# qutech/filter_functions

Hardware: AMD Instinct MI355X
Metric: filter-function elements/sec (n_seg*n_omega*n_nops*d^2) at d=4 (higher is better)
Workload: dtype f64

## Files before the change

filter_functions_amd/csrc/post.hip:

```cpp
#include <algorithm>

#include <cstdlib>

#include "ffk_internal.h"

namespace ffk {
namespace {

__global__ void reduce_chunks_kernel(const cplx* __restrict__ Ypart, int chunks, size_t slab,
                                     cplx* __restrict__ Bt) {
    const size_t e = static_cast<size_t>(blockIdx.x)*blockDim.x + threadIdx.x;
    if (e >= slab) return;
    cplx acc = Ypart[e];
    for (int c = 1; c < chunks; ++c) {
        const cplx v = Ypart[static_cast<size_t>(c)*slab + e];
        acc.re += v.re;
        acc.im += v.im;
    }
    Bt[e] = acc;
}

__global__ __launch_bounds__(64) void basis_compact_kernel(const cplx* __restrict__ basis, int d,
                                                           int* __restrict__ nnz,
                                                           int* __restrict__ rows,
// ... 328 lines not shown
    const int w = blockIdx.x*blockDim.x + threadIdx.x;
    if (w >= W) return;
    for (long long ab = blockIdx.z; ab < static_cast<long long>(A)*A; ab += gridDim.z) {
        const int a = static_cast<int>(ab / A), b = static_cast<int>(ab % A);
        for (long long kl = blockIdx.y; kl < static_cast<long long>(N)*N; kl += gridDim.y) {
            const int k = static_cast<int>(kl / N), l = static_cast<int>(kl % N);
            const cplx x = R[(static_cast<size_t>(a)*N + k)*W + w];
            const cplx y = R[(static_cast<size_t>(b)*N + l)*W + w];
            const double rr = x.re*y.re;
            const double ii = x.im*y.im;
            const double ri = x.re*y.im;
            const double ir = x.im*y.re;
            cplx v;
            v.re = rr + ii;
            v.im = ri - ir;
            F[((((static_cast<size_t>(a)*A + b)*N + k)*N + l))*W + w] = v;
        }
    }
}

constexpr int kInfidSlots = 1024, kInfidThreads = 256;
constexpr int kInfidPer = kInfidSlots/kInfidThreads;

template <int J0, int JN, typename LoadF, typename LoadS>
__device__ __forceinline__ void infid_batch(int base, int W, const double* __restrict__ omega, LoadF Fat, LoadS Sat,
                                            double (&acc)[kInfidPer], double* red = nullptr) {
    const int lane = threadIdx.x & 63;
    cplx f[kInfidPer], sp[kInfidPer];
    double om[kInfidPer];
#pragma unroll
    for (int j = J0; j < J0 + JN; ++j) {
        const int w = base + static_cast<int>(threadIdx.x) + kInfidThreads*j;
        const int wc = w < W ? w : W - 1;
        f[j] = Fat(wc);
        sp[j] = Sat(wc);
        om[j] = omega[wc];
    }
#pragma unroll
    for (int j = J0; j < J0 + JN; ++j) {
        const int w = base + static_cast<int>(threadIdx.x) + kInfidThreads*j;
        const double i0 = f[j].re*sp[j].re - f[j].im*sp[j].im;
        double i1 = __shfl_down(i0, 1, 64), o1 = __shfl_down(om[j], 1, 64);
        if (lane == 63 && w + 1 < W) {
            const cplx f1 = Fat(w + 1), s1 = Sat(w + 1);
            i1 = f1.re*s1.re - f1.im*s1.im;
            o1 = omega[w + 1];
        }
        if (w < W - 1) {
            if (red != nullptr) red[threadIdx.x + kInfidThreads*j] += (i1 + i0)*(o1 - om[j]);
            else acc[j] += (i1 + i0)*(o1 - om[j]);
        }
    }
}

template <bool FROM_REGISTERS = true>
__device__ __forceinline__ void infid_finish(double* red, const double (&acc)[kInfidPer], int d, double* out) {
    static_assert(kInfidPer == 4 && kInfidThreads == 256, "the tree below is written for 4 slots per thread, 4 wavefronts");
    double sl[kInfidPer];
#pragma unroll
    for (int j = 0; j < kInfidPer; ++j) sl[j] = FROM_REGISTERS ? acc[j] : red[threadIdx.x + kInfidThreads*j];
    double x = (sl[0] + sl[2]) + (sl[1] + sl[3]);
    __syncthreads();
    red[threadIdx.x] = x;
    __syncthreads();
    if (threadIdx.x < 128) red[threadIdx.x] = x = x + red[threadIdx.x + 128];
    __syncthreads();
    if (threadIdx.x < 64) {
        x = x + red[threadIdx.x + 64];
#pragma unroll
        for (int off = 32; off > 0; off >>= 1) x = x + __shfl_down(x, off, 64);
        if (threadIdx.x == 0) *out = (x/2.0)/(2.0*3.141592653589793*d);
    }
}

template <bool SHARDED>
__device__ __forceinline__ void infid_element(const cplx* __restrict__ F, int A, int W,
                                              const cplx* __restrict__ S, int s_ndim,
                                              const double* __restrict__ omega,
                                              const int32_t* __restrict__ idx, int n_idx,
                                              int d, int shard_width,
                                              double* __restrict__ infid, const int p) {
    __shared__ double red[kInfidSlots];
    __builtin_amdgcn_s_setprio(3);
    int ia, ib;
    const cplx* Sp;
    if (s_ndim == 3) {
        ia = idx[p / n_idx];
        ib = idx[p % n_idx];
        Sp = S + static_cast<size_t>(p)*W;
    } else {
        ia = ib = idx[p];
        Sp = S + (s_ndim == 2 ? static_cast<size_t>(p)*W : 0);
    }
    const cplx* Fp = F + (static_cast<size_t>(ia)*A + ib)*(SHARDED ? shard_width : W);
    auto Fat = [&](int w) -> cplx {
        if (SHARDED) {
            const int r = w / shard_width, wl = w - r*shard_width;
            return Fp[static_cast<size_t>(r)*A*A*shard_width + wl];
        }
        return Fp[w];
    };
    auto Sat = [&](int w) -> cplx { return Sp[w]; };
    double acc[kInfidPer];
#pragma unroll
    for (int j = 0; j < kInfidPer; ++j) red[threadIdx.x + kInfidThreads*j] = 0.0;
    for (int base = 0; base < W - 1; base += kInfidSlots) {
        infid_batch<0, kInfidPer>(base, W, omega, Fat, Sat, acc, red);
        asm volatile("" ::: "memory");
    }
    infid_finish<false>(red, acc, d, infid + p);
}

template <bool SHARDED>
__global__ __launch_bounds__(kInfidThreads) void infid_kernel(const cplx* __restrict__ F, int A, int W,
                                                              const cplx* __restrict__ S, int s_ndim,
                                                              const double* __restrict__ omega,
                                                              const int32_t* __restrict__ idx, int n_idx,
                                                              int d, int shard_width,
                                                              double* __restrict__ infid) {
    infid_element<SHARDED>(F, A, W, S, s_ndim, omega, idx, n_idx, d, shard_width, infid, blockIdx.x);
}

__global__ __launch_bounds__(kInfidThreads) void infid_pulses_kernel(const cplx* __restrict__ F, int A, int W,
                                                                     const cplx* __restrict__ S, int s_ndim,
                                                                     const double* __restrict__ omega,
                                                                     const int32_t* __restrict__ idx, int n_idx,
                                                                     int d, int nout, double* __restrict__ infid) {
    const size_t q = blockIdx.y;
    infid_element<false>(F + q*A*A*W, A, W, S, s_ndim, omega, idx, n_idx, d, 0, infid + q*nout, blockIdx.x);
}
// ... 2 lines not shown
__global__ __launch_bounds__(kInfidThreads) void infid_host_spectrum_kernel(
    const cplx* __restrict__ F, int A, int W, const cplx* __restrict__ S, int s_ndim,
    const double* __restrict__ omega, const int32_t* __restrict__ idx, int n_idx, int d,
    double* __restrict__ infid) {
    __shared__ double red[kInfidSlots];
    extern __shared__ __attribute__((aligned(16))) unsigned char stage_raw[];
    cplx* sl = reinterpret_cast<cplx*>(stage_raw);
    const int p = blockIdx.x;
    int ia, ib;
    const cplx* Sp;
    if (s_ndim == 3) {
        ia = idx[p / n_idx];
        ib = idx[p % n_idx];
        Sp = S + static_cast<size_t>(p)*W;
    } else {
        ia = ib = idx[p];
        Sp = S + (s_ndim == 2 ? static_cast<size_t>(p)*W : 0);
    }
    const cplx* Fp = F + (static_cast<size_t>(ia)*A + ib)*W;
    constexpr int kLoads = kInfidStage/kInfidThreads + 1;
    double acc[kInfidPer];
#pragma unroll
    for (int j = 0; j < kInfidPer; ++j) acc[j] = 0.0;
    for (int s0 = 0; s0 < W - 1; s0 += kInfidStage) {
        const int n = min(kInfidStage + 1, W - s0);
        cplx v[kLoads];
#pragma unroll
        for (int k = 0; k < kLoads; ++k) {
            const int i = threadIdx.x + kInfidThreads*k;
            v[k] = i < n ? Sp[s0 + i] : cplx{0.0, 0.0};
        }
#pragma unroll
        for (int k = 0; k < kLoads; ++k) {
            const int i = threadIdx.x + kInfidThreads*k;
            if (i < n) sl[i] = v[k];
        }
        __syncthreads();
        auto Fat = [&](int w) -> cplx { return Fp[w]; };
        auto Sat = [&](int w) -> cplx { return sl[w - s0]; };
        const int bend = min(W - 1, s0 + kInfidStage);
        for (int base = s0; base < bend; base += kInfidSlots) infid_batch<0, kInfidPer>(base, W, omega, Fat, Sat, acc);
        __syncthreads();
    }
    infid_finish(red, acc, d, infid + p);
}

}

hipError_t launch_reduce_chunks(const cplx* Ypart, int chunks, size_t slab, cplx* Bt,
                                hipStream_t stream) {
    const int block = 256;
    hipLaunchKernelGGL(reduce_chunks_kernel, dim3(static_cast<unsigned>((slab + block - 1)/block)),
                       dim3(block), 0, stream, Ypart, chunks, slab, Bt);
    return hipGetLastError();
}

size_t expand_workspace_bytes(int N, int d) {
    const size_t dd = static_cast<size_t>(d)*d;
    return align_up(sizeof(int)*N) + align_up(sizeof(int)*N*dd) + align_up(sizeof(cplx)*N*dd);
}

namespace {
struct CompactWs {
    int* nnz;
// ... 41 lines not shown
    const cplx* b = Ypart + static_cast<size_t>(a)*dd*W + w;
    const int n = nnz[k];
    const int* rk = rows + static_cast<size_t>(k)*dd;
    const cplx* vk = vals + static_cast<size_t>(k)*dd;
    auto summed = [&](int e) {
        cplx acc = b[static_cast<size_t>(e)*W];
        for (int z = 1; z < chunks; ++z) {
            const cplx v = b[z*slab + static_cast<size_t>(e)*W];
            acc.re += v.re;
            acc.im += v.im;
        }
        return acc;
    };
    cplx acc0 = {0.0, 0.0}, acc1 = {0.0, 0.0};
    int q = 0;
    for (; q + 1 < n; q += 2) {
        cmac(acc0, vk[q], summed(rk[q]));
        cmac(acc1, vk[q + 1], summed(rk[q + 1]));
    }
    if (q < n) cmac(acc0, vk[q], summed(rk[q]));
    R[(static_cast<size_t>(a)*N + k)*W + w] = {acc0.re + acc1.re, acc0.im + acc1.im};
}

__device__ __forceinline__ void expand_ff_tile(const cplx* __restrict__ Ypart, int chunks, size_t slab,
                                               const int* __restrict__ nnz, const int* __restrict__ rows,
                                               const cplx* __restrict__ vals, int N, int dd, int W, int A,
                                               int kt, cplx* __restrict__ R, cplx* __restrict__ F) {
    extern __shared__ __attribute__((aligned(16))) unsigned char lds_raw[];
    cplx* rl = reinterpret_cast<cplx*>(lds_raw);
    __builtin_amdgcn_s_setprio(3);
    cplx* ys = rl + static_cast<size_t>(A)*N*16;
    const int wl = threadIdx.x & 15;
    const int kl = (threadIdx.x >> 4) % kt, al = (threadIdx.x >> 4) / kt;
    const int at = (blockDim.x >> 4) / kt;
    const int w = blockIdx.x*16 + wl;
    const int wc = w < W ? w : W - 1;
    for (int idx = threadIdx.x >> 4; idx < A*dd; idx += blockDim.x >> 4) {
        const cplx* b = Ypart + static_cast<size_t>(idx)*W + wc;
        cplx acc = b[0];
        for (int z = 1; z < chunks; ++z) {
            const cplx v = b[z*slab];
            acc.re += v.re;
            acc.im += v.im;
        }
        ys[static_cast<size_t>(idx)*16 + wl] = acc;
    }
    __syncthreads();
    for (int a = al; a < A; a += at) {
        const cplx* ya = ys + static_cast<size_t>(a)*dd*16 + wl;
        for (int k = kl; k < N; k += kt) {
            const int n = nnz[k];
            const int* rk = rows + static_cast<size_t>(k)*dd;
            const cplx* vk = vals + static_cast<size_t>(k)*dd;
            auto summed = [&](int e) { return ya[e*16]; };
            cplx acc0 = {0.0, 0.0}, acc1 = {0.0, 0.0};
            int q = 0;
            for (; q + 1 < n; q += 2) {
                cmac(acc0, vk[q], summed(rk[q]));
                cmac(acc1, vk[q + 1], summed(rk[q + 1]));
            }
            if (q < n) cmac(acc0, vk[q], summed(rk[q]));
            const cplx r = {acc0.re + acc1.re, acc0.im + acc1.im};
            rl[(static_cast<size_t>(a)*N + k)*16 + wl] = r;
            if (w < W) R[(static_cast<size_t>(a)*N + k)*W + w] = r;
        }
    }
    __syncthreads();
    if (w >= W) return;
    const int npairs = A*(A + 1)/2;
    const int lanes = blockDim.x >> 4;
    for (int p = threadIdx.x >> 4; p < npairs; p += lanes) {
        int a = 0, rem = p;
        while (rem >= A - a) {
            rem -= A - a;
            ++a;
        }
        const int b = a + rem;
        const cplx* ra = rl + static_cast<size_t>(a)*N*16 + wl;
        const cplx* rb = rl + static_cast<size_t>(b)*N*16 + wl;
        cplx acc = {0.0, 0.0};
        for (int k = 0; k < N; ++k) cmac_conj(acc, ra[k*16], rb[k*16]);
        if (a == b) acc.im = 0.0;
        F[(static_cast<size_t>(a)*A + b)*W + w] = acc;
        if (a != b) F[(static_cast<size_t>(b)*A + a)*W + w] = {acc.re, -acc.im};
    }
}

__global__ __launch_bounds__(256) void expand_ff_kernel(const cplx* __restrict__ Ypart, int chunks,
                                                         size_t slab, const int* __restrict__ nnz,
// ... 5 lines not shown
}

__global__ __launch_bounds__(256) void expand_ff_pulses_kernel(const cplx* __restrict__ Ypart, int chunks,
                                                                size_t slab, const int* __restrict__ nnz,
                                                                const int* __restrict__ rows,
                                                                const cplx* __restrict__ vals, int N, int dd,
                                                                int W, int A, int kt, cplx* __restrict__ R,
                                                                cplx* __restrict__ F) {
    const size_t p = blockIdx.y;
    expand_ff_tile(Ypart + p*chunks*slab, chunks, slab, nnz, rows, vals, N, dd, W, A, kt,
                   R + p*A*N*W, F + p*A*A*W);
}

bool expand_ff_supported(int A, int N) {
    return static_cast<size_t>(A)*2*N*16*sizeof(cplx) <= 128*1024;
}

hipError_t launch_expand_ff(const cplx* Ypart, int chunks, size_t slab, int A, int N, int d, int W,
                            cplx* R, cplx* F, void* ws, hipStream_t stream) {
    if (!expand_ff_supported(A, N)) return hipErrorInvalidValue;
    const CompactWs cw = slice_compact_ws(ws, N, d);
    const int kt = N >= 16 ? 16 : (N >= 8 ? 8 : 4);
    const int at = std::max(1, std::min(A, 16/kt));
    const size_t lds = static_cast<size_t>(A)*(N + d*d)*16*sizeof(cplx);
    if (lds > 160*1024) return hipErrorInvalidValue;
    if (lds > 48*1024) {
        hipError_t err = hipFuncSetAttribute(reinterpret_cast<const void*>(expand_ff_kernel),
                                             hipFuncAttributeMaxDynamicSharedMemorySize,
                                             static_cast<int>(lds));
        if (err != hipSuccess) return err;
    }
    hipLaunchKernelGGL(expand_ff_kernel, dim3((W + 15)/16), dim3(16*kt*at), lds, stream, Ypart,
                       chunks, slab, cw.nnz, cw.rows, cw.vals, N, d*d, W, A, kt, R, F);
    return hipGetLastError();
}

hipError_t launch_expand_ff_pulses(const cplx* Ypart, int chunks, size_t slab, int A, int N, int d, int W,
                                   int P, cplx* R, cplx* F, void* ws, hipStream_t stream) {
    if (!expand_ff_supported(A, N) || P < 1 || P > 65535) return hipErrorInvalidValue;
    const CompactWs cw = slice_compact_ws(ws, N, d);
    const int kt = N >= 16 ? 16 : (N >= 8 ? 8 : 4);
    const int at = std::max(1, std::min(A, 16/kt));
    const size_t lds = static_cast<size_t>(A)*(N + d*d)*16*sizeof(cplx);
    if (lds > 160*1024) return hipErrorInvalidValue;
    if (lds > 48*1024) {
        hipError_t err = hipFuncSetAttribute(reinterpret_cast<const void*>(expand_ff_pulses_kernel),
                                             hipFuncAttributeMaxDynamicSharedMemorySize,
                                             static_cast<int>(lds));
        if (err != hipSuccess) return err;
    }
    hipLaunchKernelGGL(expand_ff_pulses_kernel, dim3((W + 15)/16, P), dim3(16*kt*at), lds, stream, Ypart,
                       chunks, slab, cw.nnz, cw.rows, cw.vals, N, d*d, W, A, kt, R, F);
    return hipGetLastError();
}

__global__ __launch_bounds__(256) void expand_lds_kernel(const cplx* __restrict__ Ypart, int chunks,
                                                         size_t slab, const int* __restrict__ nnz,
                                                         const int* __restrict__ rows,
                                                         const cplx* __restrict__ vals, int N, int dd,
                                                         int W, cplx* __restrict__ R, int want_sparse) {
    extern __shared__ __attribute__((aligned(16))) unsigned char lds_raw[];
    if (want_sparse >= 0 && basis_is_sparse(nnz, N, dd) != (want_sparse != 0)) return;
    cplx* yl = reinterpret_cast<cplx*>(lds_raw);
    const int wl = threadIdx.x & 15, kl = threadIdx.x >> 4;
    const int a = blockIdx.y;
    const int w = blockIdx.x*16 + wl;
// ... 140 lines not shown
}

hipError_t launch_filter_function_weighted(const cplx* R, int A, int N, int W, const cplx* M,
                                           double scale, cplx* F, hipStream_t stream) {
    const int block = 128;
    hipLaunchKernelGGL(ff_weighted_kernel,
                       dim3((W + block - 1)/block, grid_axis(static_cast<long long>(A)*A)),
                       dim3(block), 0, stream, R, A, N, W, M, scale, F);
    return hipGetLastError();
}

size_t infidelity_workspace_bytes(int W, int n_idx, int s_ndim) {
    (void)W;
    (void)n_idx;
    (void)s_ndim;
    return 256;
}

hipError_t launch_infidelity_pulses(const cplx* F, int A, int W, int P, const cplx* S, int s_ndim,
                                    const double* omega, const int32_t* idx, int n_idx, int d, double* infid,
                                    hipStream_t stream) {
    const int nout = s_ndim == 3 ? n_idx*n_idx : n_idx;
    if (P < 1 || P > 65535) return hipErrorInvalidValue;
    hipLaunchKernelGGL(infid_pulses_kernel, dim3(nout, P), dim3(kInfidThreads), 0, stream, F, A, W, S, s_ndim,
                       omega, idx, n_idx, d, nout, infid);
    return hipGetLastError();
}

hipError_t launch_infidelity(const cplx* F, int A, int W, const cplx* S, int s_ndim,
                             const double* omega, const int32_t* idx, int n_idx, int d,
                             int shard_width, double* infid, void* ws, hipStream_t stream,
                             bool spectrum_on_host) {
    (void)ws;
    const int nout = s_ndim == 3 ? n_idx*n_idx : n_idx;
    if (spectrum_on_host && (shard_width <= 0 || shard_width >= W)) {
        const int lds = static_cast<int>(sizeof(cplx))*(kInfidStage + 1);
        hipError_t err = hipFuncSetAttribute(reinterpret_cast<const void*>(infid_host_spectrum_kernel),
                                             hipFuncAttributeMaxDynamicSharedMemorySize, lds);
        if (err != hipSuccess) return err;
        hipLaunchKernelGGL(infid_host_spectrum_kernel, dim3(nout), dim3(kInfidThreads), lds, stream, F, A, W, S,
                           s_ndim, omega, idx, n_idx, d, infid);
        return hipGetLastError();
    }
    if (shard_width > 0 && shard_width < W)
        hipLaunchKernelGGL(infid_kernel<true>, dim3(nout), dim3(kInfidThreads), 0, stream, F, A, W, S, s_ndim, omega,
                           idx, n_idx, d, shard_width, infid);
    else
        hipLaunchKernelGGL(infid_kernel<false>, dim3(nout), dim3(kInfidThreads), 0, stream, F, A, W, S, s_ndim, omega,
                           idx, n_idx, d, shard_width, infid);
    return hipGetLastError();
}

}
```

filter_functions_amd/csrc/prep.hip:

```cpp
#include "ffk_internal.h"

namespace ffk {
namespace {

template <int D>
__device__ void prologue_segment(const cplx (*V)[D], cplx (*Q)[D], cplx (*T)[D], cplx (*BV)[D],
                                 int g, int lane, const double* __restrict__ eigvals,
                                 const cplx* __restrict__ n_opers,
                                 const double* __restrict__ n_coeffs,
                                 const double* __restrict__ dt, const double* __restrict__ t, int G,
                                 int A, double* __restrict__ segtab, cplx* __restrict__ Tc,
                                 cplx* __restrict__ ops, cplx* __restrict__ n_opers_transformed,
                                 cplx* __restrict__ eigvecs_propagated, bool with_noise_ops = true,
                                 cplx* __restrict__ wfold = nullptr) {
    constexpr int S = seg_stride(D);
    double* st = segtab + static_cast<size_t>(g)*S;
    if (lane == 0) {
        st[0] = dt[g];
        st[1] = t[g];
    }
    cplx eb = {1.0, 0.0};
    for (int e = lane; e < D*D; e += 64) {
        const double dE = eigvals[static_cast<size_t>(g)*D + e / D] - eigvals[static_cast<size_t>(g)*D + e % D];
        double sb, cb;
        sincos_pi(0.5*(dE*dt[g]), &sb, &cb);
        st[seg_rec(e)] = dE;
        st[seg_rec(e) + 1] = sb;
        st[seg_rec(e) + 2] = cb;
        st[seg_rec(e) + 3] = 0.0;
        eb = {cb, sb};
    }
    if (lane < 2) st[2 + lane] = 0.0;
    for (int e = 4 + 4*D*D + lane; e < S; e += 64) st[e] = 0.0;

    for (int e = lane; e < D*D; e += 64) {
        const int m = e / D, j = e % D;
        cplx acc = {0.0, 0.0};
#pragma unroll
        for (int k = 0; k < D; ++k) cmac_conj(acc, V[k][m], Q[k][j]);
        T[m][j] = acc;
        Tc[static_cast<size_t>(g)*D*D + e] = {acc.re, -acc.im};
        ops[static_cast<size_t>(g)*(1 + A)*D*D + e] = acc;
        if (eigvecs_propagated)
            eigvecs_propagated[static_cast<size_t>(g)*D*D + j*D + m] = {acc.re, -acc.im};
    }
    __syncthreads();

    if (!with_noise_ops) return;
    const bool fold = D == 4 && wfold != nullptr;
    if (fold) {
        if (lane < D*D) Q[lane / D][lane % D] = eb;
        __syncthreads();
    }
    for (int a = 0; a < A; ++a) {
        const cplx* B = n_opers + static_cast<size_t>(a)*D*D;
        const double s = n_coeffs ? n_coeffs[static_cast<size_t>(a)*G + g] : 1.0;
        for (int e = lane; e < D*D; e += 64) {
            const int i = e / D, n = e % D;
            cplx acc = {0.0, 0.0};
#pragma unroll
            for (int k = 0; k < D; ++k) cmac(acc, B[i*D + k], V[k][n]);
            BV[i][n] = acc;
        }
        __syncthreads();
        cplx bbar = {0.0, 0.0};
        for (int e = lane; e < D*D; e += 64) {
            const int m = e / D, n = e % D;
            cplx acc = {0.0, 0.0};
#pragma unroll
            for (int k = 0; k < D; ++k) cmac_conj(acc, V[k][m], BV[k][n]);
            acc.re *= s;
            acc.im *= s;
            ops[(static_cast<size_t>(g)*(1 + A) + 1 + a)*D*D + e] = acc;
            if (n_opers_transformed)
                n_opers_transformed[(static_cast<size_t>(a)*G + g)*D*D + e] = acc;
            if (fold) bbar = acc;
        }
        __syncthreads();
        if (fold) {
            if (lane < D*D) BV[lane / D][lane % D] = bbar;
            __syncthreads();
            if constexpr (D == 4) {
                const int m = lane >> 4, n = (lane >> 2) & 3, j = lane & 3;
                const cplx et = cmul(Q[m][n], T[n][j]);
                const cplx w = cmul(BV[m][n], et);
                wfold[(static_cast<size_t>(g)*A + a)*64 + n*16 + m*4 + j] = w;
// ... 71 lines not shown
        const int i = e / D, n = e % D;
        cplx acc = {0.0, 0.0};
#pragma unroll
        for (int k = 0; k < D; ++k) cmac(acc, B[i*D + k], V[k][n]);
        BV[i][n] = acc;
    }
    __syncthreads();
    for (int e = lane; e < D*D; e += 64) {
        const int m = e / D, n = e % D;
        cplx acc = {0.0, 0.0};
#pragma unroll
        for (int k = 0; k < D; ++k) cmac_conj(acc, V[k][m], BV[k][n]);
        acc.re *= s;
        acc.im *= s;
        ops[(static_cast<size_t>(g)*(1 + A) + 1 + a)*D*D + e] = acc;
        if (n_opers_transformed)
            n_opers_transformed[(static_cast<size_t>(a)*G + g)*D*D + e] = acc;
    }
}

constexpr int kNoiseOpsKernelMinD = 12;
inline bool split_noise_ops(int d, int A) { return d >= kNoiseOpsKernelMinD && A >= 2 && A <= 65535; }

template <int D>
__device__ __forceinline__ void apply_prologue_segment(
    const cplx* __restrict__ Qloc, const cplx* __restrict__ totals, int G, int L,
    cplx* __restrict__ Qout, const double* __restrict__ eigvals, const cplx* __restrict__ eigvecs,
    const cplx* __restrict__ n_opers, const double* __restrict__ n_coeffs,
    const double* __restrict__ dt, const double* __restrict__ t, int A,
    double* __restrict__ segtab, cplx* __restrict__ Tc, cplx* __restrict__ ops,
    bool with_noise_ops, cplx* __restrict__ wfold, const int g) {
    __builtin_amdgcn_s_setprio(3);
    __shared__ cplx E[2][D][D];
    __shared__ cplx M[D][D];
    __shared__ cplx V[D][D];
    __shared__ cplx Q[D][D];
    __shared__ cplx T[D][D];
    __shared__ cplx BV[D][D];
    constexpr int kBatch = 16;
    constexpr bool kTree = D <= 8;
    extern __shared__ __attribute__((aligned(16))) unsigned char tot_raw[];
    cplx (*tot)[D][D] = reinterpret_cast<cplx (*)[D][D]>(tot_raw);
    const int lane = threadIdx.x;
    const int c = g / L;
    for (int e = lane; e < D*D; e += 64) E[0][e / D][e % D] = {(e / D == e % D) ? 1.0 : 0.0, 0.0};
    int b = 0;
    if constexpr (kTree) {
        constexpr int DD = D*D, PER = 64/DD;
        for (int e = lane; e < c*DD; e += 64) (&tot[0][0][0])[e] = totals[e];
        __syncthreads();
        int n = c;
        while (n > 1) {
            const int pairs = n >> 1;
            for (int j0 = 0; j0 < pairs; j0 += PER) {
                const int jj = j0 + lane/DD, e = lane % DD, i = e / D, k = e % D;
                const bool act = lane < PER*DD && jj < pairs;
                cplx acc = {0.0, 0.0};
                if (act) {
#pragma unroll
                    for (int x = 0; x < D; ++x) cmac(acc, tot[2*jj + 1][i][x], tot[2*jj][x][k]);
                }
                __syncthreads();
                if (act) tot[jj][i][k] = acc;
                __syncthreads();
            }
            if (n & 1) {
                const cplx* from = &tot[n - 1][0][0] + (lane < DD ? lane : 0);
                const double carry_re = from->re, carry_im = from->im;
                __syncthreads();
                if (lane < DD) (&tot[pairs][0][0])[lane] = {carry_re, carry_im};
                __syncthreads();
            }
// ... 3 lines not shown
            for (int e = lane; e < DD; e += 64) E[0][e / D][e % D] = tot[0][e / D][e % D];
            __syncthreads();
        }
    } else {
    for (int kb = 0; kb < c; kb += kBatch) {
        const int nb = min(kBatch, c - kb);
        __syncthreads();
        for (int e = lane; e < nb*D*D; e += 64)
            (&tot[0][0][0])[e] = totals[static_cast<size_t>(kb)*D*D + e];
        __syncthreads();
        for (int k = 0; k < nb; ++k) {
            for (int e = lane; e < D*D; e += 64) {
                const int i = e / D, j = e % D;
                cplx acc = {0.0, 0.0};
#pragma unroll
                for (int x = 0; x < D; ++x) cmac(acc, tot[k][i][x], E[b][x][j]);
                E[b ^ 1][i][j] = acc;
            }
            __syncthreads();
            b ^= 1;
        }
    }
    }
    for (int e = lane; e < D*D; e += 64) M[e / D][e % D] = Qloc[static_cast<size_t>(g + 1)*D*D + e];
    if (g == 0)
        for (int e = lane; e < D*D; e += 64) Qout[e] = {(e / D == e % D) ? 1.0 : 0.0, 0.0};
    __syncthreads();
    for (int e = lane; e < D*D; e += 64) {
        const int i = e / D, j = e % D;
        cplx acc = {0.0, 0.0};
#pragma unroll
        for (int x = 0; x < D; ++x) cmac(acc, M[i][x], E[b][x][j]);
        Qout[static_cast<size_t>(g + 1)*D*D + e] = acc;
    }
    if (segtab == nullptr) return;
    __syncthreads();
    if (g % L == 0) {
        for (int e = lane; e < D*D; e += 64) Q[e / D][e % D] = E[b][e / D][e % D];
    } else {
        for (int e = lane; e < D*D; e += 64) M[e / D][e % D] = Qloc[static_cast<size_t>(g)*D*D + e];
        __syncthreads();
        for (int e = lane; e < D*D; e += 64) {
            const int i = e / D, j = e % D;
            cplx acc = {0.0, 0.0};
#pragma unroll
            for (int x = 0; x < D; ++x) cmac(acc, M[i][x], E[b][x][j]);
            Q[i][j] = acc;
        }
    }
    for (int e = lane; e < D*D; e += 64) V[e / D][e % D] = eigvecs[static_cast<size_t>(g)*D*D + e];
    __syncthreads();
    prologue_segment<D>(V, Q, T, BV, g, lane, eigvals, n_opers, n_coeffs, dt, t, G, A, segtab, Tc,
                        ops, nullptr, nullptr, with_noise_ops, wfold);
}

template <int D>
__global__ __launch_bounds__(64) void apply_prologue_kernel(
    const cplx* __restrict__ Qloc, const cplx* __restrict__ totals, int G, int L,
    cplx* __restrict__ Qout, const double* __restrict__ eigvals, const cplx* __restrict__ eigvecs,
    const cplx* __restrict__ n_opers, const double* __restrict__ n_coeffs,
    const double* __restrict__ dt, const double* __restrict__ t, int A,
    double* __restrict__ segtab, cplx* __restrict__ Tc, cplx* __restrict__ ops,
    const cplx* __restrict__ basis, int* __restrict__ nnz, int* __restrict__ rows,
    cplx* __restrict__ vals, bool with_noise_ops, cplx* __restrict__ wfold) {
    if (static_cast<int>(blockIdx.x) >= G) {
        basis_compact_one(basis, D, static_cast<int>(blockIdx.x) - G, threadIdx.x, nnz, rows, vals);
        return;
    }
    apply_prologue_segment<D>(Qloc, totals, G, L, Qout, eigvals, eigvecs, n_opers, n_coeffs, dt, t, A, segtab, Tc,
                              ops, with_noise_ops, wfold, blockIdx.x);
}

template <int D>
__global__ __launch_bounds__(64) void apply_prologue_pulses_kernel(
    const cplx* __restrict__ Qloc, const cplx* __restrict__ totals, int G, int L, int nchunks,
    cplx* __restrict__ Qout, const double* __restrict__ eigvals, const cplx* __restrict__ eigvecs,
// ... 135 lines not shown
        FFK_CASE(2) FFK_CASE(3) FFK_CASE(4) FFK_CASE(5) FFK_CASE(6) FFK_CASE(7) FFK_CASE(8)
#undef FFK_CASE
        default:
            return hipErrorInvalidValue;
    }
    return hipGetLastError();
}

hipError_t launch_apply_prologue_compact(const cplx* Qloc, const cplx* totals, int G, int d, cplx* Q,
                                         const double* eigvals, const cplx* eigvecs,
                                         const cplx* n_opers, const double* n_coeffs,
                                         const double* dt, const double* t, int A, double* segtab,
                                         cplx* Tc, cplx* ops, const cplx* basis, int N, void* ews,
                                         hipStream_t stream, cplx* wfold) {
    const int L = front_chunk(d);
    int* nnz = nullptr;
    int* rows = nullptr;
    cplx* vals = nullptr;
    int extra = 0;
    if (basis) {
        expand_workspace_slices(ews, N, d, &nnz, &rows, &vals);
        extra = N;
    }
    switch (d) {
#define FFK_CASE(D)                                                                              \
    case D:                                                                                      \
        if (D > 8) {    \
            hipError_t e = hipFuncSetAttribute(reinterpret_cast<const void*>(apply_prologue_kernel<D>), \
                                               hipFuncAttributeMaxDynamicSharedMemorySize,       \
                                               static_cast<int>(sizeof(cplx)*D*D*16));           \
            if (e != hipSuccess) return e;                                                       \
        }                                                                                        \
        hipLaunchKernelGGL(apply_prologue_kernel<D>, dim3(G + extra), dim3(64),                  \
                           sizeof(cplx)*D*D*(D <= 8 ? (G + L - 1)/L : 16), stream, Qloc,         \
                           totals, G, L, Q, eigvals, eigvecs, n_opers, n_coeffs, dt, t, A,       \
                           segtab, Tc, ops, basis, nnz, rows, vals, !split_noise_ops(D, A),      \
                           D == 4 ? wfold : nullptr);                                            \
        if (split_noise_ops(D, A))                                                               \
            hipLaunchKernelGGL(noise_ops_kernel<D>, dim3(G, A), dim3(64), 0, stream, eigvecs,    \
                               n_opers, n_coeffs, G, A, ops, nullptr);                           \
        break;
        FFK_CASE(2) FFK_CASE(3) FFK_CASE(4) FFK_CASE(5) FFK_CASE(6) FFK_CASE(7) FFK_CASE(8)
        FFK_CASE(9) FFK_CASE(10) FFK_CASE(11) FFK_CASE(12) FFK_CASE(13) FFK_CASE(14)
        FFK_CASE(15) FFK_CASE(16)
#undef FFK_CASE
        default:
            return hipErrorInvalidValue;
    }
    if (d == 8 && wfold != nullptr) return launch_fold_w8(segtab, ops, G, A, wfold, stream);
    return hipGetLastError();
}

hipError_t launch_apply_prologue_compact_pulses(const cplx* Qloc, const cplx* totals, int G, int P, int d,
                                                cplx* Q, const double* eigvals, const cplx* eigvecs,
                                                const cplx* n_opers, const double* n_coeffs, const double* dt,
                                                const double* t, int A, double* segtab, cplx* Tc, cplx* ops,
                                                const cplx* basis, int N, void* ews, hipStream_t stream,
                                                cplx* wfold) {
    const int L = front_chunk(d);
    const int nchunks = (G + L - 1)/L;
    if (P < 1 || P > 65535 || !basis) return hipErrorInvalidValue;
    int* nnz = nullptr;
    int* rows = nullptr;
    cplx* vals = nullptr;
    expand_workspace_slices(ews, N, d, &nnz, &rows, &vals);
    switch (d) {
#define FFK_CASE(D)                                                                              \
    case D:                                                                                      \
        if (D > 8) {                                                                             \
            hipError_t e = hipFuncSetAttribute(reinterpret_cast<const void*>(apply_prologue_pulses_kernel<D>), \
                                               hipFuncAttributeMaxDynamicSharedMemorySize,       \
                                               static_cast<int>(sizeof(cplx)*D*D*16));           \
            if (e != hipSuccess) return e;                                                       \
        }                                                                                        \
        hipLaunchKernelGGL(apply_prologue_pulses_kernel<D>, dim3(G + N, P), dim3(64),            \
                           sizeof(cplx)*D*D*(D <= 8 ? nchunks : 16), stream, Qloc, totals, G, L, \
                           nchunks, Q, eigvals, eigvecs, n_opers, n_coeffs, dt, t, A, segtab, Tc, \
                           ops, basis, nnz, rows, vals, D == 4 ? wfold : nullptr);               \
        break;
        FFK_CASE(2) FFK_CASE(3) FFK_CASE(4) FFK_CASE(5) FFK_CASE(6) FFK_CASE(7) FFK_CASE(8)
        FFK_CASE(9) FFK_CASE(10) FFK_CASE(11) FFK_CASE(12) FFK_CASE(13) FFK_CASE(14)
        FFK_CASE(15) FFK_CASE(16)
#undef FFK_CASE
        default:
            return hipErrorInvalidValue;
    }
    if (d == 8 && wfold != nullptr) return launch_fold_w8(segtab, ops, P*G, A, wfold, stream);
    return hipGetLastError();
}

hipError_t launch_apply_prologue(const cplx* Qloc, const cplx* totals, int G, int d, cplx* Q,
                                 const double* eigvals, const cplx* eigvecs, const cplx* n_opers,
                                 const double* n_coeffs, const double* dt, const double* t, int A,
                                 double* segtab, cplx* Tc, cplx* ops, hipStream_t stream) {
    return launch_apply_prologue_compact(Qloc, totals, G, d, Q, eigvals, eigvecs, n_opers, n_coeffs,
                                         dt, t, A, segtab, Tc, ops, nullptr, 0, nullptr, stream);
}

hipError_t launch_basis_transformed(const cplx* Tc, const cplx* basis, int G, int N, int d,
// ... 31 lines not shown
```

Before: 880.1 billion.

## Batch global loads ahead and stage sparse lists and boundaries in LDS

```diff
diff --git a/filter_functions_amd/csrc/post.hip b/filter_functions_amd/csrc/post.hip
--- a/filter_functions_amd/csrc/post.hip
+++ b/filter_functions_amd/csrc/post.hip
@@ -374,33 +374,59 @@
 constexpr int kInfidSlots = 1024, kInfidThreads = 256;
 constexpr int kInfidPer = kInfidSlots/kInfidThreads;
 
-template <int J0, int JN, typename LoadF, typename LoadS>
+__device__ __forceinline__ double infid_integrand(const cplx f, const cplx s) { return f.re*s.re - f.im*s.im; }
+
+constexpr int kInfidBoundary = 2*2*17;
+
+template <typename LoadF, typename LoadS>
 __device__ __forceinline__ void infid_batch(int base, int W, const double* __restrict__ omega, LoadF Fat, LoadS Sat,
-                                            double (&acc)[kInfidPer], double* red = nullptr) {
+                                            double (&acc)[kInfidPer], double* bnd, double* red = nullptr) {
+    static_assert(kInfidPer == 4 && kInfidThreads == 256, "16 boundary points: 4 slots x 4 wavefronts");
     const int lane = threadIdx.x & 63;
+    const int wave = static_cast<int>(threadIdx.x) >> 6;
     cplx f[kInfidPer], sp[kInfidPer];
-    double om[kInfidPer];
-#pragma unroll
-    for (int j = J0; j < J0 + JN; ++j) {
+    double om[kInfidPer], i0[kInfidPer];
+#pragma unroll
+    for (int j = 0; j < kInfidPer; ++j) {
         const int w = base + static_cast<int>(threadIdx.x) + kInfidThreads*j;
         const int wc = w < W ? w : W - 1;
         f[j] = Fat(wc);
         sp[j] = Sat(wc);
         om[j] = omega[wc];
     }
-#pragma unroll
-    for (int j = J0; j < J0 + JN; ++j) {
-        const int w = base + static_cast<int>(threadIdx.x) + kInfidThreads*j;
-        const double i0 = f[j].re*sp[j].re - f[j].im*sp[j].im;
-        double i1 = __shfl_down(i0, 1, 64), o1 = __shfl_down(om[j], 1, 64);
-        if (lane == 63 && w + 1 < W) {
-            const cplx f1 = Fat(w + 1), s1 = Sat(w + 1);
-            i1 = f1.re*s1.re - f1.im*s1.im;
-            o1 = omega[w + 1];
-        }
-        if (w < W - 1) {
-            if (red != nullptr) red[threadIdx.x + kInfidThreads*j] += (i1 + i0)*(o1 - om[j]);
-            else acc[j] += (i1 + i0)*(o1 - om[j]);
+    __builtin_amdgcn_sched_barrier(0);
+    const int par = (base/kInfidSlots) & 1;
+    double* mine = bnd + par*34 + 2*wave;
+#pragma unroll
+    for (int j = 0; j < kInfidPer; ++j) {
+        i0[j] = infid_integrand(f[j], sp[j]);
+        if (lane == 0) {
+            mine[8*j] = i0[j];
+            mine[8*j + 1] = om[j];
+        }
+    }
+    __syncthreads();
+    const bool last = threadIdx.x == kInfidThreads - 1;
+    if (last && base > 0) {
+        const double* prev = mine + (par ? -34 : 34);
+        const double i1 = mine[-6], o1 = mine[-5], ic = prev[26], oc = prev[27];
+        if (red != nullptr) red[threadIdx.x + kInfidThreads*(kInfidPer - 1)] += (i1 + ic)*(o1 - oc);
+        else acc[kInfidPer - 1] += (i1 + ic)*(o1 - oc);
+    }
+    const int left = W - 1 - base - static_cast<int>(threadIdx.x);
+#pragma unroll
+    for (int j = 0; j < kInfidPer; ++j) {
+        double i1 = __shfl_down(i0[j], 1, 64), o1 = __shfl_down(om[j], 1, 64);
+        if (lane == 63) {
+            i1 = mine[8*j + 2];
+            o1 = mine[8*j + 3];
+        }
+        if (j == kInfidPer - 1 && last) {
+            mine[26] = i0[j];
+            mine[27] = om[j];
+        } else if (kInfidThreads*j < left) {
+            if (red != nullptr) red[threadIdx.x + kInfidThreads*j] += (i1 + i0[j])*(o1 - om[j]);
+            else acc[j] += (i1 + i0[j])*(o1 - om[j]);
         }
     }
 }
@@ -433,6 +459,8 @@
                                               int d, int shard_width,
                                               double* __restrict__ infid, const int p) {
     __shared__ double red[kInfidSlots];
+    extern __shared__ __attribute__((aligned(16))) unsigned char bnd_raw[];
+    double* bnd = reinterpret_cast<double*>(bnd_raw);
     __builtin_amdgcn_s_setprio(3);
     int ia, ib;
     const cplx* Sp;
@@ -456,8 +484,8 @@
     double acc[kInfidPer];
 #pragma unroll
     for (int j = 0; j < kInfidPer; ++j) red[threadIdx.x + kInfidThreads*j] = 0.0;
-    for (int base = 0; base < W - 1; base += kInfidSlots) {
-        infid_batch<0, kInfidPer>(base, W, omega, Fat, Sat, acc, red);
+    for (int base = 0; base < W; base += kInfidSlots) {
+        infid_batch(base, W, omega, Fat, Sat, acc, bnd, red);
         asm volatile("" ::: "memory");
     }
     infid_finish<false>(red, acc, d, infid + p);
@@ -506,7 +534,8 @@
     double acc[kInfidPer];
 #pragma unroll
     for (int j = 0; j < kInfidPer; ++j) acc[j] = 0.0;
-    for (int s0 = 0; s0 < W - 1; s0 += kInfidStage) {
+    double* bnd = red + kInfidThreads;
+    for (int s0 = 0; s0 < W; s0 += kInfidStage) {
         const int n = min(kInfidStage + 1, W - s0);
         cplx v[kLoads];
 #pragma unroll
@@ -522,8 +551,8 @@
         __syncthreads();
         auto Fat = [&](int w) -> cplx { return Fp[w]; };
         auto Sat = [&](int w) -> cplx { return sl[w - s0]; };
-        const int bend = min(W - 1, s0 + kInfidStage);
-        for (int base = s0; base < bend; base += kInfidSlots) infid_batch<0, kInfidPer>(base, W, omega, Fat, Sat, acc);
+        const int bend = min(W, s0 + kInfidStage);
+        for (int base = s0; base < bend; base += kInfidSlots) infid_batch(base, W, omega, Fat, Sat, acc, bnd);
         __syncthreads();
     }
     infid_finish(red, acc, d, infid + p);
@@ -611,6 +640,11 @@
     R[(static_cast<size_t>(a)*N + k)*W + w] = {acc0.re + acc1.re, acc0.im + acc1.im};
 }
 
+__host__ __device__ constexpr bool expand_ff_lists_in_lds(int N, int dd) { return N*dd <= 1024; }
+__host__ __device__ constexpr size_t expand_ff_lds_bytes(int A, int N, int dd) {
+    return static_cast<size_t>(A)*(N + dd)*16*sizeof(cplx) +
+           (expand_ff_lists_in_lds(N, dd) ? static_cast<size_t>(N)*dd*(sizeof(cplx) + sizeof(int)) + sizeof(int)*N : 0);
+}
 __device__ __forceinline__ void expand_ff_tile(const cplx* __restrict__ Ypart, int chunks, size_t slab,
                                                const int* __restrict__ nnz, const int* __restrict__ rows,
                                                const cplx* __restrict__ vals, int N, int dd, int W, int A,
@@ -624,36 +658,93 @@
     const int at = (blockDim.x >> 4) / kt;
     const int w = blockIdx.x*16 + wl;
     const int wc = w < W ? w : W - 1;
-    for (int idx = threadIdx.x >> 4; idx < A*dd; idx += blockDim.x >> 4) {
-        const cplx* b = Ypart + static_cast<size_t>(idx)*W + wc;
-        cplx acc = b[0];
-        for (int z = 1; z < chunks; ++z) {
-            const cplx v = b[z*slab];
-            acc.re += v.re;
-            acc.im += v.im;
-        }
-        ys[static_cast<size_t>(idx)*16 + wl] = acc;
+    const bool lists_staged = expand_ff_lists_in_lds(N, dd);
+    const int nl = N*dd;
+    cplx* vals_l = ys + static_cast<size_t>(A)*dd*16;
+    int* rows_l = reinterpret_cast<int*>(vals_l + nl);
+    int* nnz_l = rows_l + nl;
+    const int tid = threadIdx.x, nthreads = blockDim.x;
+    int row0 = 0, nnz0 = 0;
+    double val0_re = 0.0, val0_im = 0.0;
+    if (lists_staged) {
+        const int e = tid < nl ? tid : nl - 1;
+        row0 = rows[e];
+        val0_re = vals[e].re;
+        val0_im = vals[e].im;
+        nnz0 = nnz[tid < N ? tid : N - 1];
+    }
+    {
+        constexpr int kFly = 8;
+        const int groups = nthreads >> 4, g0 = tid >> 4, entries = A*dd;
+        const int ne = (entries + groups - 1)/groups;
+        const int total = ne*chunks;
+        int li = 0, lz = 0;
+        int si = 0, sz = 0;
+        double acc_re = 0.0, acc_im = 0.0;
+        for (int q0 = 0; q0 < total; q0 += kFly) {
+            cplx v[kFly];
+#pragma unroll
+            for (int u = 0; u < kFly; ++u) {
+                const int idx = min(g0 + li*groups, entries - 1);
+                v[u] = Ypart[lz*slab + static_cast<size_t>(idx)*W + wc];
+                if (q0 + u + 1 < total) {
+                    if (++lz == chunks) {
+                        lz = 0;
+                        ++li;
+                    }
+                }
+            }
+#pragma unroll
+            for (int u = 0; u < kFly; ++u) {
+                if (q0 + u < total) {
+                    acc_re = sz == 0 ? v[u].re : acc_re + v[u].re;
+                    acc_im = sz == 0 ? v[u].im : acc_im + v[u].im;
+                    if (++sz == chunks) {
+                        const int idx = g0 + si*groups;
+                        if (idx < entries) ys[static_cast<size_t>(idx)*16 + wl] = {acc_re, acc_im};
+                        sz = 0;
+                        ++si;
+                    }
+                }
+            }
+        }
+    }
+    if (lists_staged) {
+        if (tid < nl) {
+            rows_l[tid] = row0;
+            vals_l[tid] = {val0_re, val0_im};
+        }
+        if (tid < N) nnz_l[tid] = nnz0;
+        for (int e = tid + nthreads; e < nl; e += nthreads) {
+            rows_l[e] = rows[e];
+            vals_l[e] = vals[e];
+        }
+        for (int e = tid + nthreads; e < N; e += nthreads) nnz_l[e] = nnz[e];
     }
     __syncthreads();
-    for (int a = al; a < A; a += at) {
-        const cplx* ya = ys + static_cast<size_t>(a)*dd*16 + wl;
-        for (int k = kl; k < N; k += kt) {
-            const int n = nnz[k];
-            const int* rk = rows + static_cast<size_t>(k)*dd;
-            const cplx* vk = vals + static_cast<size_t>(k)*dd;
-            auto summed = [&](int e) { return ya[e*16]; };
-            cplx acc0 = {0.0, 0.0}, acc1 = {0.0, 0.0};
-            int q = 0;
-            for (; q + 1 < n; q += 2) {
-                cmac(acc0, vk[q], summed(rk[q]));
-                cmac(acc1, vk[q + 1], summed(rk[q + 1]));
+    auto expand = [&](const int* __restrict__ nz, const int* __restrict__ rw, const cplx* __restrict__ vl) {
+        for (int a = al; a < A; a += at) {
+            const cplx* ya = ys + static_cast<size_t>(a)*dd*16 + wl;
+            for (int k = kl; k < N; k += kt) {
+                const int n = nz[k];
+                const int* rk = rw + static_cast<size_t>(k)*dd;
+                const cplx* vk = vl + static_cast<size_t>(k)*dd;
+                auto summed = [&](int e) { return ya[e*16]; };
+                cplx acc0 = {0.0, 0.0}, acc1 = {0.0, 0.0};
+                int q = 0;
+                for (; q + 1 < n; q += 2) {
+                    cmac(acc0, vk[q], summed(rk[q]));
+                    cmac(acc1, vk[q + 1], summed(rk[q + 1]));
+                }
+                if (q < n) cmac(acc0, vk[q], summed(rk[q]));
+                const cplx r = {acc0.re + acc1.re, acc0.im + acc1.im};
+                rl[(static_cast<size_t>(a)*N + k)*16 + wl] = r;
+                if (w < W) R[(static_cast<size_t>(a)*N + k)*W + w] = r;
             }
-            if (q < n) cmac(acc0, vk[q], summed(rk[q]));
-            const cplx r = {acc0.re + acc1.re, acc0.im + acc1.im};
-            rl[(static_cast<size_t>(a)*N + k)*16 + wl] = r;
-            if (w < W) R[(static_cast<size_t>(a)*N + k)*W + w] = r;
-        }
-    }
+        }
+    };
+    if (lists_staged) expand(nnz_l, rows_l, vals_l);
+    else expand(nnz, rows, vals);
     __syncthreads();
     if (w >= W) return;
     const int npairs = A*(A + 1)/2;
@@ -705,7 +796,7 @@
     const CompactWs cw = slice_compact_ws(ws, N, d);
     const int kt = N >= 16 ? 16 : (N >= 8 ? 8 : 4);
     const int at = std::max(1, std::min(A, 16/kt));
-    const size_t lds = static_cast<size_t>(A)*(N + d*d)*16*sizeof(cplx);
+    const size_t lds = expand_ff_lds_bytes(A, N, d*d);
     if (lds > 160*1024) return hipErrorInvalidValue;
     if (lds > 48*1024) {
         hipError_t err = hipFuncSetAttribute(reinterpret_cast<const void*>(expand_ff_kernel),
@@ -724,7 +815,7 @@
     const CompactWs cw = slice_compact_ws(ws, N, d);
     const int kt = N >= 16 ? 16 : (N >= 8 ? 8 : 4);
     const int at = std::max(1, std::min(A, 16/kt));
-    const size_t lds = static_cast<size_t>(A)*(N + d*d)*16*sizeof(cplx);
+    const size_t lds = expand_ff_lds_bytes(A, N, d*d);
     if (lds > 160*1024) return hipErrorInvalidValue;
     if (lds > 48*1024) {
         hipError_t err = hipFuncSetAttribute(reinterpret_cast<const void*>(expand_ff_pulses_kernel),
@@ -911,8 +1002,8 @@
                                     hipStream_t stream) {
     const int nout = s_ndim == 3 ? n_idx*n_idx : n_idx;
     if (P < 1 || P > 65535) return hipErrorInvalidValue;
-    hipLaunchKernelGGL(infid_pulses_kernel, dim3(nout, P), dim3(kInfidThreads), 0, stream, F, A, W, S, s_ndim,
-                       omega, idx, n_idx, d, nout, infid);
+    hipLaunchKernelGGL(infid_pulses_kernel, dim3(nout, P), dim3(kInfidThreads), kInfidBoundary*sizeof(double), stream,
+                       F, A, W, S, s_ndim, omega, idx, n_idx, d, nout, infid);
     return hipGetLastError();
 }
 
@@ -932,12 +1023,12 @@
         return hipGetLastError();
     }
     if (shard_width > 0 && shard_width < W)
-        hipLaunchKernelGGL(infid_kernel<true>, dim3(nout), dim3(kInfidThreads), 0, stream, F, A, W, S, s_ndim, omega,
-                           idx, n_idx, d, shard_width, infid);
+        hipLaunchKernelGGL(infid_kernel<true>, dim3(nout), dim3(kInfidThreads), kInfidBoundary*sizeof(double), stream,
+                           F, A, W, S, s_ndim, omega, idx, n_idx, d, shard_width, infid);
     else
-        hipLaunchKernelGGL(infid_kernel<false>, dim3(nout), dim3(kInfidThreads), 0, stream, F, A, W, S, s_ndim, omega,
-                           idx, n_idx, d, shard_width, infid);
-    return hipGetLastError();
-}
-
-}
+        hipLaunchKernelGGL(infid_kernel<false>, dim3(nout), dim3(kInfidThreads), kInfidBoundary*sizeof(double), stream,
+                           F, A, W, S, s_ndim, omega, idx, n_idx, d, shard_width, infid);
+    return hipGetLastError();
+}
+
+}
diff --git a/filter_functions_amd/csrc/prep.hip b/filter_functions_amd/csrc/prep.hip
--- a/filter_functions_amd/csrc/prep.hip
+++ b/filter_functions_amd/csrc/prep.hip
@@ -4,7 +4,7 @@
 namespace {
 
 template <int D>
-__device__ void prologue_segment(const cplx (*V)[D], cplx (*Q)[D], cplx (*T)[D], cplx (*BV)[D],
+__device__ __forceinline__ void prologue_segment(const cplx (*V)[D], cplx (*Q)[D], cplx (*T)[D], cplx (*BV)[D],
                                  int g, int lane, const double* __restrict__ eigvals,
                                  const cplx* __restrict__ n_opers,
                                  const double* __restrict__ n_coeffs,
@@ -12,18 +12,25 @@
                                  int A, double* __restrict__ segtab, cplx* __restrict__ Tc,
                                  cplx* __restrict__ ops, cplx* __restrict__ n_opers_transformed,
                                  cplx* __restrict__ eigvecs_propagated, bool with_noise_ops = true,
-                                 cplx* __restrict__ wfold = nullptr) {
+                                 cplx* __restrict__ wfold = nullptr, const bool ahead = false,
+                                 const double ev_m = 0.0, const double ev_n = 0.0, const double dt_g = 0.0,
+                                 const double t_g = 0.0, const unsigned ops_off = 0) {
+    extern __shared__ __attribute__((aligned(16))) unsigned char ahead_raw[];
+    const cplx* ops_l = reinterpret_cast<const cplx*>(ahead_raw + ops_off);
+    const double* coeffs_l = reinterpret_cast<const double*>(ops_l + static_cast<size_t>(A)*D*D);
     constexpr int S = seg_stride(D);
     double* st = segtab + static_cast<size_t>(g)*S;
+    const double dtg = ahead ? dt_g : dt[g];
     if (lane == 0) {
-        st[0] = dt[g];
-        st[1] = t[g];
+        st[0] = dtg;
+        st[1] = ahead ? t_g : t[g];
     }
     cplx eb = {1.0, 0.0};
     for (int e = lane; e < D*D; e += 64) {
-        const double dE = eigvals[static_cast<size_t>(g)*D + e / D] - eigvals[static_cast<size_t>(g)*D + e % D];
+        const double dE = ahead ? ev_m - ev_n
+                                : eigvals[static_cast<size_t>(g)*D + e / D] - eigvals[static_cast<size_t>(g)*D + e % D];
         double sb, cb;
-        sincos_pi(0.5*(dE*dt[g]), &sb, &cb);
+        sincos_pi(0.5*(dE*dtg), &sb, &cb);
         st[seg_rec(e)] = dE;
         st[seg_rec(e) + 1] = sb;
         st[seg_rec(e) + 2] = cb;
@@ -53,15 +60,19 @@
         __syncthreads();
     }
     for (int a = 0; a < A; ++a) {
-        const cplx* B = n_opers + static_cast<size_t>(a)*D*D;
-        const double s = n_coeffs ? n_coeffs[static_cast<size_t>(a)*G + g] : 1.0;
-        for (int e = lane; e < D*D; e += 64) {
-            const int i = e / D, n = e % D;
-            cplx acc = {0.0, 0.0};
-#pragma unroll
-            for (int k = 0; k < D; ++k) cmac(acc, B[i*D + k], V[k][n]);
-            BV[i][n] = acc;
-        }
+        const double s = ahead ? coeffs_l[a]
+                               : (n_coeffs ? n_coeffs[static_cast<size_t>(a)*G + g] : 1.0);
+        auto times_v = [&](const cplx* __restrict__ B) {
+            for (int e = lane; e < D*D; e += 64) {
+                const int i = e / D, n = e % D;
+                cplx acc = {0.0, 0.0};
+#pragma unroll
+                for (int k = 0; k < D; ++k) cmac(acc, B[i*D + k], V[k][n]);
+                BV[i][n] = acc;
+            }
+        };
+        if (ahead) times_v(ops_l + static_cast<size_t>(a)*D*D);
+        else times_v(n_opers + static_cast<size_t>(a)*D*D);
         __syncthreads();
         cplx bbar = {0.0, 0.0};
         for (int e = lane; e < D*D; e += 64) {
@@ -179,6 +190,13 @@
 constexpr int kNoiseOpsKernelMinD = 12;
 inline bool split_noise_ops(int d, int A) { return d >= kNoiseOpsKernelMinD && A >= 2 && A <= 65535; }
 
+__host__ __device__ constexpr bool prologue_noise_ops_in_lds(int d, int A) { return d <= 8 && A >= 1 && A*d*d <= 1024; }
+inline size_t apply_prologue_lds_bytes(int d, int nchunks, int A, bool with_noise_ops) {
+    const size_t dd = static_cast<size_t>(d)*d;
+    return sizeof(cplx)*dd*(d <= 8 ? nchunks : 16) +
+           (with_noise_ops && prologue_noise_ops_in_lds(d, A) ? sizeof(cplx)*dd*A + sizeof(double)*A : 0);
+}
+
 template <int D>
 __device__ __forceinline__ void apply_prologue_segment(
     const cplx* __restrict__ Qloc, const cplx* __restrict__ totals, int G, int L,
@@ -196,15 +214,70 @@
     __shared__ cplx BV[D][D];
     constexpr int kBatch = 16;
     constexpr bool kTree = D <= 8;
+    constexpr int kDD = D*D;
+    constexpr int kTotAhead = 4;
     extern __shared__ __attribute__((aligned(16))) unsigned char tot_raw[];
     cplx (*tot)[D][D] = reinterpret_cast<cplx (*)[D][D]>(tot_raw);
     const int lane = threadIdx.x;
     const int c = g / L;
+    const bool ahead_ops = kTree && segtab != nullptr && with_noise_ops && prologue_noise_ops_in_lds(D, A);
+    double ev_m = 0.0, ev_n = 0.0, dt_g = 0.0, t_g = 0.0;
+    if constexpr (kTree) {
+        const int e = lane < kDD ? lane : kDD - 1;
+        const int ntot = c*kDD;
+        double q0_re = 0.0, q0_im = 0.0, vv_re = 0.0, vv_im = 0.0;
+        double op0_re = 0.0, op0_im = 0.0, co0 = 1.0;
+        double tot_re[kTotAhead], tot_im[kTotAhead];
+#pragma unroll
+        for (int k = 0; k < kTotAhead; ++k) {
+            const int x = lane + 64*k;
+            const cplx* src = totals + (x < ntot ? x : (ntot > 0 ? ntot - 1 : 0));
+            tot_re[k] = src->re;
+            tot_im[k] = src->im;
+        }
+        const double q1_re = Qloc[static_cast<size_t>(g + 1)*kDD + e].re;
+        const double q1_im = Qloc[static_cast<size_t>(g + 1)*kDD + e].im;
+        cplx* ops_l = reinterpret_cast<cplx*>(tot_raw) + static_cast<size_t>((G + L - 1)/L)*kDD;
+        double* co_l = reinterpret_cast<double*>(ops_l + static_cast<size_t>(A)*kDD);
+        if (segtab != nullptr) {
+            q0_re = Qloc[static_cast<size_t>(g)*kDD + e].re;
+            q0_im = Qloc[static_cast<size_t>(g)*kDD + e].im;
+            vv_re = eigvecs[static_cast<size_t>(g)*kDD + e].re;
+            vv_im = eigvecs[static_cast<size_t>(g)*kDD + e].im;
+            ev_m = eigvals[static_cast<size_t>(g)*D + e / D];
+            ev_n = eigvals[static_cast<size_t>(g)*D + e % D];
+            dt_g = dt[g];
+            t_g = t[g];
+            if (ahead_ops) {
+                op0_re = n_opers[lane < A*kDD ? lane : A*kDD - 1].re;
+                op0_im = n_opers[lane < A*kDD ? lane : A*kDD - 1].im;
+                if (n_coeffs) co0 = n_coeffs[static_cast<size_t>(lane < A ? lane : A - 1)*G + g];
+            }
+        }
+        asm volatile("" :: "v"(tot_re[0]), "v"(tot_im[0]), "v"(tot_re[1]), "v"(tot_im[1]), "v"(tot_re[2]),
+                     "v"(tot_im[2]), "v"(tot_re[3]), "v"(tot_im[3]), "v"(q1_re), "v"(q1_im), "v"(q0_re), "v"(q0_im),
+                     "v"(vv_re), "v"(vv_im), "v"(op0_re), "v"(op0_im), "v"(co0), "v"(ev_m), "v"(ev_n), "s"(dt_g),
+                     "s"(t_g));
+#pragma unroll
+        for (int k = 0; k < kTotAhead; ++k)
+            if (lane + 64*k < ntot) (&tot[0][0][0])[lane + 64*k] = {tot_re[k], tot_im[k]};
+        if (lane < kDD) {
+            M[lane / D][lane % D] = {q1_re, q1_im};
+            T[lane / D][lane % D] = {q0_re, q0_im};
+            V[lane / D][lane % D] = {vv_re, vv_im};
+        }
+        if (ahead_ops) {
+            if (lane < A*kDD) ops_l[lane] = {op0_re, op0_im};
+            if (lane < A) co_l[lane] = co0;
+            for (int x = lane + 64; x < A*kDD; x += 64) ops_l[x] = n_opers[x];
+            for (int x = lane + 64; x < A; x += 64) co_l[x] = n_coeffs ? n_coeffs[static_cast<size_t>(x)*G + g] : 1.0;
+        }
+    }
     for (int e = lane; e < D*D; e += 64) E[0][e / D][e % D] = {(e / D == e % D) ? 1.0 : 0.0, 0.0};
     int b = 0;
     if constexpr (kTree) {
         constexpr int DD = D*D, PER = 64/DD;
-        for (int e = lane; e < c*DD; e += 64) (&tot[0][0][0])[e] = totals[e];
+        for (int e = lane + 64*kTotAhead; e < c*DD; e += 64) (&tot[0][0][0])[e] = totals[e];
         __syncthreads();
         int n = c;
         while (n > 1) {
@@ -254,7 +327,8 @@
         }
     }
     }
-    for (int e = lane; e < D*D; e += 64) M[e / D][e % D] = Qloc[static_cast<size_t>(g + 1)*D*D + e];
+    if constexpr (!kTree)
+        for (int e = lane; e < D*D; e += 64) M[e / D][e % D] = Qloc[static_cast<size_t>(g + 1)*D*D + e];
     if (g == 0)
         for (int e = lane; e < D*D; e += 64) Qout[e] = {(e / D == e % D) ? 1.0 : 0.0, 0.0};
     __syncthreads();
@@ -270,7 +344,8 @@
     if (g % L == 0) {
         for (int e = lane; e < D*D; e += 64) Q[e / D][e % D] = E[b][e / D][e % D];
     } else {
-        for (int e = lane; e < D*D; e += 64) M[e / D][e % D] = Qloc[static_cast<size_t>(g)*D*D + e];
+        for (int e = lane; e < D*D; e += 64)
+            M[e / D][e % D] = kTree ? T[e / D][e % D] : Qloc[static_cast<size_t>(g)*D*D + e];
         __syncthreads();
         for (int e = lane; e < D*D; e += 64) {
             const int i = e / D, j = e % D;
@@ -280,10 +355,17 @@
             Q[i][j] = acc;
         }
     }
-    for (int e = lane; e < D*D; e += 64) V[e / D][e % D] = eigvecs[static_cast<size_t>(g)*D*D + e];
-    __syncthreads();
-    prologue_segment<D>(V, Q, T, BV, g, lane, eigvals, n_opers, n_coeffs, dt, t, G, A, segtab, Tc,
-                        ops, nullptr, nullptr, with_noise_ops, wfold);
+    if constexpr (!kTree)
+        for (int e = lane; e < D*D; e += 64) V[e / D][e % D] = eigvecs[static_cast<size_t>(g)*D*D + e];
+    __syncthreads();
+    if constexpr (kTree) {
+        prologue_segment<D>(V, Q, T, BV, g, lane, eigvals, n_opers, n_coeffs, dt, t, G, A, segtab, Tc,
+                            ops, nullptr, nullptr, with_noise_ops, wfold, ahead_ops, ev_m, ev_n, dt_g, t_g,
+                            static_cast<unsigned>(sizeof(cplx)*((G + L - 1)/L)*kDD));
+    } else {
+        prologue_segment<D>(V, Q, T, BV, g, lane, eigvals, n_opers, n_coeffs, dt, t, G, A, segtab, Tc,
+                            ops, nullptr, nullptr, with_noise_ops, wfold);
+    }
 }
 
 template <int D>
@@ -465,17 +547,18 @@
         expand_workspace_slices(ews, N, d, &nnz, &rows, &vals);
         extra = N;
     }
+    const size_t lds_bytes = apply_prologue_lds_bytes(d, (G + L - 1)/L, A, !split_noise_ops(d, A));
     switch (d) {
 #define FFK_CASE(D)                                                                              \
     case D:                                                                                      \
-        if (D > 8) {    \
+         \
+        if (D > 8 || lds_bytes > 48*1024) {                                                      \
             hipError_t e = hipFuncSetAttribute(reinterpret_cast<const void*>(apply_prologue_kernel<D>), \
                                                hipFuncAttributeMaxDynamicSharedMemorySize,       \
-                                               static_cast<int>(sizeof(cplx)*D*D*16));           \
+                                               static_cast<int>(lds_bytes));                     \
             if (e != hipSuccess) return e;                                                       \
         }                                                                                        \
-        hipLaunchKernelGGL(apply_prologue_kernel<D>, dim3(G + extra), dim3(64),                  \
-                           sizeof(cplx)*D*D*(D <= 8 ? (G + L - 1)/L : 16), stream, Qloc,         \
+        hipLaunchKernelGGL(apply_prologue_kernel<D>, dim3(G + extra), dim3(64), lds_bytes, stream, Qloc, \
                            totals, G, L, Q, eigvals, eigvecs, n_opers, n_coeffs, dt, t, A,       \
                            segtab, Tc, ops, basis, nnz, rows, vals, !split_noise_ops(D, A),      \
                            D == 4 ? wfold : nullptr);                                            \
@@ -507,17 +590,18 @@
     int* rows = nullptr;
     cplx* vals = nullptr;
     expand_workspace_slices(ews, N, d, &nnz, &rows, &vals);
+    const size_t lds_bytes = apply_prologue_lds_bytes(d, nchunks, A, true);
     switch (d) {
 #define FFK_CASE(D)                                                                              \
     case D:                                                                                      \
-        if (D > 8) {                                                                             \
+        if (D > 8 || lds_bytes > 48*1024) {                                                      \
             hipError_t e = hipFuncSetAttribute(reinterpret_cast<const void*>(apply_prologue_pulses_kernel<D>), \
                                                hipFuncAttributeMaxDynamicSharedMemorySize,       \
-                                               static_cast<int>(sizeof(cplx)*D*D*16));           \
+                                               static_cast<int>(lds_bytes));                     \
             if (e != hipSuccess) return e;                                                       \
         }                                                                                        \
         hipLaunchKernelGGL(apply_prologue_pulses_kernel<D>, dim3(G + N, P), dim3(64),            \
-                           sizeof(cplx)*D*D*(D <= 8 ? nchunks : 16), stream, Qloc, totals, G, L, \
+                           lds_bytes, stream, Qloc, totals, G, L,                                \
                            nchunks, Q, eigvals, eigvecs, n_opers, n_coeffs, dt, t, A, segtab, Tc, \
                            ops, basis, nnz, rows, vals, D == 4 ? wfold : nullptr);               \
         break;
```

After: 882.4 billion, median of 6. Within noise of the previous version (+0.3%).
